# zsyOAOA/ResShift

Hardware: AMD Instinct MI355X
Metric: images/sec (1x3x64x64 LR -> 3x256x256, 15-step ResShift sampling loop incl. VQ encode/decode) (higher is better)
Workload: dtype f16x2 encoder + UNet (hi+lo fp16 pairs, 3 MFMAs per product: fp32-class) + f16 decoder (parity policy); 1 GPU; realsr_swinunet_realesrgan256: batch 32/GPU x 1 GPU, 1x3x64x64 LR -> 3x256x256, 15 steps, random-init weights; precision_policy=parity, parallelism=dp1 (batch sharded, one RCCL weight broadcast, no data-path collective)

## Files before the change

### include/resshift_hip.h

```cpp
#ifndef RESSHIFT_HIP_H
#define RESSHIFT_HIP_H
#include <stddef.h>
#include <stdint.h>

#ifdef __cplusplus
extern "C" {
#endif

#define RS_PREC_F16 0
#define RS_PREC_F32 1
#define RS_PREC_SPLIT 2
#define RS_MAX_LEVELS 8
#define RS_MAX_STEPS 64
#define RS_MAX_ROWS 64

typedef struct rs_engine rs_engine;

typedef struct rs_unet_config {
    int image_size, in_channels, model_channels, out_channels;
    int n_levels;
    int channel_mult[RS_MAX_LEVELS];
    int num_res_blocks[RS_MAX_LEVELS];
    int n_attn_res;
    int attention_resolutions[RS_MAX_LEVELS];
// ... 117 lines not shown
int rs_debug_enable(rs_engine* e, int on);
int rs_debug_count(rs_engine* e);
int rs_debug_info(rs_engine* e, int i, char* name, int name_cap, int* dims_bchw);
int rs_debug_fetch(rs_engine* e, int i, float* out_nchw_dev, void* stream);
int rs_debug_fetch_rows(rs_engine* e, int i, int b0, int nb, float* out_nchw_dev, void* stream);

int rs_op_conv2d(const void* x0, const void* x1, const float* w_ref_host, const float* bias_host, const void* res, void* y,
                 int B, int Hs, int Ws, int C0, int C1, int Cout, int KH, int KW, int stride, int pad_t, int pad_l, int Ho,
                 int Wo, int up, int act, int in_prec, int out_prec, int force_direct, void* stream);
int rs_op_conv2d_bench(const void* x0, const void* w_packed_dev, const float* bias_dev, const void* res, void* y, int B, int Hs,
                       int Ws, int Cin, int Cout, int KH, int KW, int stride, int pad, int Ho, int Wo, int up, int act, int in_prec,
                       int out_prec, int reps, float* ms_out, void* stream);
int rs_op_conv3x3_halo(const void* x, const float* coef_dev, int act_in, const float* w_ref_host, const float* bias_host, const void* res,
                       void* y, int B, int H, int W, int Cin, int Cout, int prec, float* ystats_dev, void* stream);
int rs_op_conv3x3_wino(const void* x, const float* coef_dev, int act_in, const float* w_ref_host, const float* bias_host, const void* res,
                       void* y, int B, int H, int W, int Cin, int Cout, float* ystats_dev, int reps, float* ms_out, void* stream);
int rs_op_conv3x3_halo_stats_px(int B, int H, int W, int Cin, int Cout, int prec);
int rs_op_gemm_nt(const void* a, const void* b, const float* bias_dev, void* y, int nz, int M, int N, int K, float scale,
                  int in_prec, int out_prec, void* stream);
int rs_op_groupnorm(const void* x, void* y, const float* gamma_host, const float* beta_host, const float* film_dev, int B, int HW,
                    int C, int groups, float eps, int act, int prec, void* stream);
int rs_op_window_attention(const void* qkv, void* out, const float* bias_table_host , int B, int H, int W,
                           int heads, int shift, int prec, void* stream);
int rs_op_window_attention_qkv(const void* x, const void* wqkv_dev, const float* bqkv_dev, const void* wproj_dev, const float* bproj_dev,
                               const void* res, void* out, const float* table_host, int B, int H, int W, int heads, int shift, void* stream);
int rs_op_window_attention_qkv_split(const void* x, const void* wqkv_dev, const float* bqkv_dev, const void* wproj_dev, const float* bproj_dev,
                                     const void* res, void* out, const float* table_host, const float* xcoef_dev, int B, int H, int W, int heads,
                                     int shift, void* stream);
int rs_op_ae_flash_attention(const void* q, const void* k, const void* vt, const float* bv_dev, void* o, int nz, int T, int C, void* stream);
int rs_op_ae_flash_attention_split(const void* q, const void* k, const void* vt, const float* bv_dev, void* o, int nz, int T, int C, void* stream);
int rs_op_swin_mlp(const void* x, const void* w1_dev, const float* b1_dev, const void* w2_dev, const float* b2_dev, const void* res, void* y,
// ... 16 lines not shown
```

### resshift_amd/_lib.py

```python
from __future__ import annotations

import ctypes as C
import os

import torch

HERE = os.path.dirname(os.path.abspath(__file__))
LIB_PATH = os.environ.get("RESSHIFT_HIP_LIB") or os.path.join(HERE, "libresshift_hip.so")

RS_PREC_F16 = 0
RS_PREC_F32 = 1
RS_PREC_SPLIT = 2
RS_MAX_LEVELS = 8
RS_MAX_STEPS = 64
RS_MAX_ROWS = 64


class UNetConfig(C.Structure):
    _fields_ = [
        ("image_size", C.c_int), ("in_channels", C.c_int), ("model_channels", C.c_int), ("out_channels", C.c_int),
        ("n_levels", C.c_int),
        ("channel_mult", C.c_int * RS_MAX_LEVELS),
        ("num_res_blocks", C.c_int * RS_MAX_LEVELS),
        ("n_attn_res", C.c_int),
# ... 100 lines not shown
    "rs_arena_bytes": (_SZ, [_P]),
    "rs_last_launch_count": (_LL, [_P]),
    "rs_profile_enable": (_I, [_P, _I]),
    "rs_profile_get": (_I, [_P, C.POINTER(C.c_double)]),
    "rs_profile_families": (_I, [_P, C.POINTER(C.c_double), _I]),
    "rs_profile_shapes": (_I, [_P, C.c_char_p, _I]),
    "rs_debug_enable": (_I, [_P, _I]),
    "rs_debug_count": (_I, [_P]),
    "rs_debug_info": (_I, [_P, _I, C.c_char_p, _I, C.POINTER(C.c_int)]),
    "rs_debug_fetch": (_I, [_P, _I, _P, _P]),
    "rs_debug_fetch_rows": (_I, [_P, _I, _I, _I, _P, _P]),
    "rs_op_conv2d": (_I, [_P, _P, _P, _P, _P, _P] + [_I] * 18 + [_P]),
    "rs_op_conv2d_bench": (_I, [_P, _P, _P, _P, _P] + [_I] * 16 + [C.POINTER(C.c_float), _P]),
    "rs_op_conv3x3_halo_stats_px": (_I, [_I, _I, _I, _I, _I, _I]),
    "rs_op_conv3x3_halo": (_I, [_P, _P, _I, _P, _P, _P, _P, _I, _I, _I, _I, _I, _I, _P, _P]),
    "rs_op_conv3x3_wino": (_I, [_P, _P, _I, _P, _P, _P, _P, _I, _I, _I, _I, _I, _P, _I, C.POINTER(C.c_float), _P]),
    "rs_op_gemm_nt": (_I, [_P, _P, _P, _P, _I, _I, _I, _I, _F, _I, _I, _P]),
    "rs_op_groupnorm": (_I, [_P, _P, _P, _P, _P, _I, _I, _I, _I, _F, _I, _I, _P]),
    "rs_op_window_attention": (_I, [_P, _P, _P, _I, _I, _I, _I, _I, _I, _P]),
    "rs_op_window_attention_qkv": (_I, [_P, _P, _P, _P, _P, _P, _P, _P, _I, _I, _I, _I, _I, _P]),
    "rs_op_window_attention_qkv_split": (_I, [_P, _P, _P, _P, _P, _P, _P, _P, _P, _I, _I, _I, _I, _I, _P]),
    "rs_op_swin_mlp": (_I, [_P, _P, _P, _P, _P, _P, _P, _I, _I, _I, _P]),
    "rs_op_ae_flash_attention": (_I, [_P, _P, _P, _P, _P, _I, _I, _I, _P]),
    "rs_op_ae_flash_attention_split": (_I, [_P, _P, _P, _P, _P, _I, _I, _I, _P]),
    "rs_op_swin_mlp_split": (_I, [_P, _P, _P, _P, _P, _P, _P, _I, _I, _I, _P]),
    "rs_op_swin_mlp_split_unembed": (_I, [_P, _P, _P, _P, _P, _P, _P, _I, _I, _I, _I, _I, _P]),
    "rs_op_softmax_rows": (_I, [_P, _P, _LL, _I, _I, _P]),
    "rs_op_vq": (_I, [_P, _P, _P, _P, _LL, _I, _I, _P]),
    "rs_op_nchw_to_nhwc": (_I, [_P, _P, _I, _I, _I, _I, _P]),
    "rs_op_nhwc_to_nchw": (_I, [_P, _P, _I, _I, _I, _I, _P]),
    "rs_op_convert": (_I, [_P, _I, _P, _I, _I, _LL, _P]),
# ... 100 lines not shown
```

### resshift_amd/csrc/engine.hip

```cpp
#include "common.h"
#include "../../include/resshift_hip.h"
#include <dlfcn.h>
#include <algorithm>
#include <array>
#include <cmath>
#include <cstdio>
#include <cstring>
#include <functional>
#include <map>
#include <string>
#include <unordered_map>
#include <vector>

extern "C" {
int rs_igemm_launch(const IGemmParams* p, int in_dt, int out_dt, int nz, hipStream_t st);
int rs_igemm_splitk_plan(int M, int Cout, int Ktot, int in_dt);
int rs_igemm4_pick(const IGemmParams* p, int in_dt, int out_dt, int nz, int* TW, int* BC);
int rs_igemm4_plan(const IGemmParams* p, int in_dt, int out_dt, int nz, int* TW, int* BC, int* SEG, int* SK);
int rs_igemm4_stats_px(const IGemmParams* p, int in_dt);
int rs_wino_plan(const IGemmParams* p, int in_dt, int out_dt, int nz);
int rs_wino_launch(const IGemmParams* p, hipStream_t st);
size_t rs_wino_weight_bytes(int Cin, int Cout);
float rs_wino_pack(const float* w_ref, int Cin, int Cout, void* dst);
int rs_wino_stats_px();
int rs_wino_tiles(const IGemmParams* p);
int rs_igemm_split_stats_px(const IGemmParams* p, int splitk);
int rs_direct_conv_launch(const DirectConvParams* p, int in_dt, int out_dt, hipStream_t st);
int rs_head_conv_launch(const void* x, int in_dt, const float* coef_dev, const float* w_dev, const float* bias_dev, float* y, int B, int H, int W, int C,
                        int ldx, int Cout, int ldy, hipStream_t st);
int rs_groupnorm_launch(const GNParams* p, int dt, int apply_slabs, hipStream_t st);
int rs_win_attn_launch(const WinAttnParams* p, int dt, hipStream_t st);
int rs_softmax_rows_launch(const float* s, void* out, int out_dt, long long nrows, int ncols, long long lds_, long long ldo, hipStream_t st);
int rs_nchw_to_nhwc_launch(const float* in, void* out, int out_dt, int B, int C, int HW, int ldo, int coff, float scale, hipStream_t st);
int rs_nhwc_to_nchw_launch(const void* in, int in_dt, float* out, int B, int C, int HW, int ldi, int coff, hipStream_t st);
int rs_axpbypcz_launch(const float* x, const float* z, const float* n, float* y, float a, float b, float c, long long cnt, hipStream_t st);
int rs_axpbypcz_rows_launch(const float* x, const float* z, const float* n, float* y, const float* a, const float* b, const float* c, long long per,
                            int B, hipStream_t st);
int rs_axpbypcz_seeded_launch(const float* x, const float* z, float* y, const float* a, const float* b, const float* c, const rs_noise_key* keys,
                              const rs_noise_key* keys_dev, const int* draw, long long per, int B, hipStream_t st);
// ... 410 lines not shown
                HostTensor t;
                if (d->second(t)) it = host.emplace(k, std::move(t)).first;
            }
        }
        if (it == host.end()) { if (build_err.empty()) build_err = "missing state_dict key: " + k; return nullptr; }
        return &it->second;
    }
    float* add_f32(const std::string& key, size_t n) {
        return (float*)blob.add(n * sizeof(float), [&](char* dst) {
            const HostTensor* t = find(key);
            if (!t) return;
            if (t->data.size() != n) { if (build_err.empty()) build_err = "bad size for " + key; return; }
            memcpy(dst, t->data.data(), n * sizeof(float));
        });
    }
    ConvW add_conv(const std::string& prefix, int Cin, int Cout, int KH, int KW, bool has_bias = true, bool force_direct = false, bool head = false) {
        ConvW c; c.Cin = Cin; c.Cout = Cout; c.KH = KH; c.KW = KW;
        c.idx = conv_count++;
        if ((int)big_w.size() < conv_count) big_w.resize(conv_count, 0);
        const int cidx = c.idx;
        c.direct = force_direct;
        c.CinP = c.direct ? Cin : (Cin + 7) / 8 * 8;
        const int CinP = c.CinP;
        const size_t K = (size_t)KH * KW * CinP, n = (size_t)KH * KW * Cin * Cout, np = K * Cout;
        const std::string wkey = prefix + ".weight";
        auto get = [&]() -> const float* {
            const HostTensor* t = find(wkey);
            if (!t) return nullptr;
            if (t->data.size() != n) { if (build_err.empty()) build_err = "bad size for " + wkey; return nullptr; }
            return t->data.data();
// ... 25 lines not shown
                    const float* w = get(); if (!w) return;
                    f16* o = (f16*)dst;
                    for (int co = 0; co < Cout; ++co)
                        for (int ci = 0; ci < Cin; ++ci)
                            for (int t = 0; t < KH * KW; ++t) {
                                f16 h, l;
                                const float wv = w[((size_t)co * Cin + ci) * KH * KW + t];
                                if (!std::isfinite(wv) || std::fabs(wv) > 60000.0f) { if (split_err.empty()) split_err = "split precision needs finite fp16-range weights: " + wkey; }
                                else if (!(std::fabs(wv) < 30.0f)) big_w[cidx] = 1;
                                rs_split(wv, h, l);
                                const size_t k = (size_t)t * CinP + ci;
                                o[(size_t)co * 2 * K + k] = h;
                                o[(size_t)co * 2 * K + K + k] = l;
                            }
                });
            static const bool wino_on = []() { const char* e = getenv("RS_WINO"); return !(e && e[0] == '0'); }();
            if (wino_on && cfg.enable_split && KH == 3 && KW == 3 && (Cin % 32) == 0 && Cin <= 640 && (Cout % 160) == 0 && Cout <= 320)
                c.ww = blob.add(rs_wino_weight_bytes(Cin, Cout), [&](char* dst) {
                    const float* w = get(); if (!w) return;
                    if (!(rs_wino_pack(w, Cin, Cout, dst) < 30.0f)) big_w[cidx] = 1;
                });
            if (cfg.enable_f32)
                c.wf = blob.add(np * 4, [&](char* dst) {
                    const float* w = get(); if (!w) return;
                    float* o = (float*)dst;
                    for (int co = 0; co < Cout; ++co)
                        for (int ci = 0; ci < Cin; ++ci)
                            for (int t = 0; t < KH * KW; ++t)
                                o[(size_t)co * K + (size_t)t * CinP + ci] = w[((size_t)co * Cin + ci) * KH * KW + t];
                });
        }
        if (head && !c.direct && KH == 3 && KW == 3 && Cout <= 4 && (Cin % 8) == 0)
// ... 242 lines not shown
        fe_out_ch = u.cond_lq ? base_chn : 0;
        int ch = u.channel_mult[0] * mc;
        const int input_ch = ch;
        {
            UBlock b; b.has_conv = true; b.level = 0; b.out_ch = ch;
            const bool two_src_unaligned = !fe_convs.empty() && (u.in_channels % 8 != 0);
            b.conv = add_conv("input_blocks.0.0", u.in_channels + fe_out_ch, ch, 3, 3, true, two_src_unaligned);
            in_blocks.push_back(b);
        }
        std::vector<int> chans{ch};
        int ds = u.image_size;
        for (int level = 0; level < u.n_levels; ++level) {
            const int mult = u.channel_mult[level];
            for (int jj = 0; jj < u.num_res_blocks[level]; ++jj) {
                UBlock b; b.level = level;
                const std::string p = "input_blocks." + std::to_string(in_blocks.size());
                b.has_res = true; b.res = add_resblock(p + ".0", ch, mult * mc, emb_ch);
                ch = mult * mc;
                if (in_attn_res(ds) && jj == 0) { b.has_swin = true; b.swin = add_basiclayer(p + ".1", ch, ds); }
                b.out_ch = ch;
                in_blocks.push_back(b); chans.push_back(ch);
            }
            if (level != u.n_levels - 1) {
                UBlock b; b.level = level + 1; b.has_down = true; b.out_ch = ch;
                b.conv = add_conv("input_blocks." + std::to_string(in_blocks.size()) + ".0.op", ch, ch, 3, 3);
                in_blocks.push_back(b); chans.push_back(ch);
                ds /= 2;
            }
        }
        skip_ch = chans;
        mid_res1 = add_resblock("middle_block.0", ch, ch, emb_ch);
        mid_swin = add_basiclayer("middle_block.1", ch, ds);
        mid_res2 = add_resblock("middle_block.2", ch, ch, emb_ch);
        for (int level = u.n_levels - 1; level >= 0; --level) {
            const int mult = u.channel_mult[level];
            for (int i = 0; i <= u.num_res_blocks[level]; ++i) {
                const int ich = chans.back(); chans.pop_back();
                UBlock b; b.level = level;
                const std::string p = "output_blocks." + std::to_string(out_blocks.size());
                h_ch.push_back(ch);
                int sub = 0;
                b.has_res = true; b.res = add_resblock(p + "." + std::to_string(sub++), ch + ich, mc * mult, emb_ch);
                ch = mc * mult;
                if (in_attn_res(ds) && i == 0) { b.has_swin = true; b.swin = add_basiclayer(p + "." + std::to_string(sub++), ch, ds); }
                if (level && i == u.num_res_blocks[level]) {
                    b.has_up = true;
                    b.conv = add_conv(p + "." + std::to_string(sub) + ".conv", ch, ch, 3, 3);
                    b.has_upf = add_upfold(p + "." + std::to_string(sub++) + ".conv", ch, b.upf);
                    ds *= 2;
                }
                b.out_ch = ch;
                out_blocks.push_back(b);
            }
        }
        out_norm = add_gn("out.0", ch);
        out_conv = add_conv("out.2", input_ch, u.out_channels, 3, 3, true, false, true);
    }
    ResBlockW add_resnet(const std::string& p, int Cin, int Cout) {
        ResBlockW r; r.Cin = Cin; r.Cout = Cout;
        r.n1 = add_gn(p + ".norm1", Cin);
        r.c1 = add_conv(p + ".conv1", Cin, Cout, 3, 3);
        r.n2 = add_gn(p + ".norm2", Cout);
        r.c2 = add_conv(p + ".conv2", Cout, Cout, 3, 3);
        r.has_skip = Cin != Cout;
        if (r.has_skip) r.skip = add_conv(p + ".nin_shortcut", Cin, Cout, 1, 1);
        return r;
    }
    AttnW add_attn(const std::string& p, int C) {
        AttnW a; a.C = C;
// ... 165 lines not shown
        if (!on || !fold || !r.has_skip || (X.dt != RS_F16S && !(X.dt == RS_F16 && on16)) || Y.dt != X.dt) return false;
        if (X.dt == RS_F16S && (big(r.skip) || big(r.c2))) return false;
        if (!r.skip.w_for(X.dt) || r.skip.KH != 1 || X.C != r.skip.CinP || (X.C % 32) || (X.ld % 8) || X.H != Y.H || X.W != Y.W) return false;
        int sk = 1, seg = 0;
        return halo_conv(r.c2, h1, Y, nullptr, &sk, &seg, true) && sk == 1 && seg == 0;
    }
    void want_stats(Exec& ex, const ConvW& w, const View& x, View& y, const View* res, int stride = 1, int pad = 1, int up = 1, bool folded = false) {
        static const bool on = []() { const char* e = getenv("RS_GN_EPI_STATS"); return !(e && e[0] == '0'); }();
        static const bool gen = []() { const char* e = getenv("RS_GN_GEN_STATS"); return !(e && e[0] == '0'); }();
        const int HW = y.H * y.W;
        y.st = nullptr; y.st2 = nullptr; y.st_prod = -1;
        if (!on || w.direct) return;
        const IGemmParams pp = conv_params(w, x, nullptr, y, stride, pad, pad, up, 0, res, 1.f);
        int spx = 0;
        bool wino = false;
        if (w.KH == 3 && stride == 1 && pad == 1 && up == 1 && halo_conv(w, x, y, res, nullptr, nullptr, folded, &wino)) spx = wino ? rs_wino_stats_px() : rs_igemm4_stats_px(&pp, x.dt);
        else if (gen && x.dt == RS_F16S && y.dt == RS_F16S && x.C == w.CinP)
            spx = rs_igemm_split_stats_px(&pp, rs_igemm_splitk_plan(pp.M, w.Cout, w.KH * w.KW * x.C, x.dt));
        if (spx <= 0 || (HW % spx)) return;
        y.stS = HW / spx; y.stld = y.C;
        y.st = ex.pool((size_t)y.B * y.stS * y.stld * 2 * sizeof(float));
        y.st_prod = ex.prod_seq++;
    }
    void gn_silu_conv3(Exec& ex, const GNW& g, const ConvW& w, const View& X, const View& Y, float eps, const float* film, const View* res,
                       const ConvW* skw = nullptr, const View* skx = nullptr) {
        static const bool fold = []() { const char* e = getenv("RS_GN_CONV_FOLD"); return !(e && e[0] == '0'); }();
        if (fold && halo_conv(w, X, Y, res, nullptr, nullptr, skw != nullptr)) {
            const float* coef = gn_coef(ex, g, X, eps, film);
            conv3(ex, w, X, Y, res, 0, coef, RS_ACT_SILU, skw, skx);
            return;
        }
// ... 1360 lines not shown
    if (!rs_igemm4_plan(&p, prec, prec, 1, &tw, &bc, &seg, &sk)) rc = fail("shape is not eligible for the halo kernel");
    else {
        p.splitk = sk;
        if (sk > 1) { (void)hipMalloc((void**)&part, (size_t)sk * p.M * Cout * sizeof(float)); p.partial = part; }
        p.ystats = ystats_dev; p.ystats_ld = Cout;
        rc = rs_igemm_launch(&p, prec, prec, 1, st);
    }
    (void)hipStreamSynchronize(st);
    if (part) (void)hipFree(part);
    if (wdev) (void)hipFree(wdev);
    if (bias) (void)hipFree(bias);
    return rc;
}

int rs_op_conv3x3_wino(const void* x, const float* coef_dev, int act_in, const float* w_ref_host, const float* bias_host, const void* res, void* y,
                       int B, int H, int W, int Cin, int Cout, float* ystats_dev, int reps, float* ms_out, void* stream) {
    hipStream_t st = (hipStream_t)stream;
    if (Cin < 32 || (Cin % 32) || Cout < 32 || (Cout % 32)) return fail("wino kernel: channels in multiples of 32");
    std::vector<char> packed(rs_wino_weight_bytes(Cin, Cout));
    const float mx = rs_wino_pack(w_ref_host, Cin, Cout, packed.data());
    if (!(mx < 30.0f)) return fail("wino kernel: |U| >= 30");
    void* wdev = dev_copy(packed.data(), packed.size());
    float* bias = bias_host ? (float*)dev_copy(bias_host, Cout * 4) : nullptr;
    IGemmParams p{};
    p.x0 = x; p.ww = wdev; p.bias = bias; p.res = res; p.y = y; p.C0 = Cin; p.ld0 = Cin; p.B = B; p.Hs = H; p.Ws = W; p.up = 1; p.Ho = H; p.Wo = W;
    p.KH = 3; p.KW = 3; p.stride = 1; p.pad_t = 1; p.pad_l = 1; p.Cout = Cout; p.ldy = Cout; p.ldres = Cout; p.M = B * H * W; p.Ktot = 9 * Cin;
    p.out_scale = 1.f; p.splitk = 1; p.xcoef = coef_dev; p.xact = act_in; p.ystats = ystats_dev; p.ystats_ld = Cout;
    int rc = 0;
    float* stamps = nullptr;
    const int ntile = rs_wino_tiles(&p);
    p.dbg = 64;
    if (const char* ab = getenv("RS_WINO_ABL")) p.dbg |= atoi(ab);
    if (getenv("RS_WINO_STAMPS")) { (void)hipMalloc((void**)&stamps, (size_t)ntile * 16 * sizeof(float)); (void)hipMemset(stamps, 0, (size_t)ntile * 16 * sizeof(float)); p.partial = stamps; }
    if (!rs_wino_plan(&p, RS_F16S, RS_F16S, 1)) rc = fail("shape is not eligible for the wino kernel");
    else {
        rc = rs_wino_launch(&p, st);
        if (rc) fail("wino launch failed");
        if (stamps) {
            (void)hipStreamSynchronize(st);
            std::vector<float> hs((size_t)ntile * 16);
            (void)hipMemcpy(hs.data(), stamps, hs.size() * sizeof(float), hipMemcpyDeviceToHost);
            double wide[16] = {}; int nw = 0;
            for (int t = 0; t < ntile; ++t) {
                for (int i = 0; i < 16; ++i) wide[i] += hs[(size_t)t * 16 + i];
                ++nw;
            }
// ... 203 lines not shown
```

### resshift_amd/csrc/wino.hip

```cpp
#include "igemm_common.h"
#include "gn_tail.h"
#include <algorithm>
#include <cmath>
#include <vector>

namespace {

using namespace igemm_detail;

typedef __attribute__((address_space(3))) void* lds_ptr_t;

__device__ __forceinline__ void wdma16s(__amdgpu_buffer_rsrc_t r, char* lds, unsigned voff, unsigned soff) {
    __builtin_amdgcn_raw_ptr_buffer_load_lds(r, (lds_ptr_t)lds, 16, voff, soff, 0, 0);
}

template <int N> __device__ __forceinline__ void wait_vm() { asm volatile("s_waitcnt vmcnt(%0)" ::"n"(N) : "memory"); }

constexpr int W_TH = 8, W_TW = 16;
constexpr int W_PITCH = 20;
constexpr int W_HROWS = (W_TH + 2) * W_PITCH;
constexpr int W_UPW = 2;
constexpr int W_NUNIT = 8 * W_UPW;
constexpr int W_HBUF = W_NUNIT * 2048;
constexpr int W_NBUF = 3;
constexpr int W_COEF = W_NBUF * W_HBUF;
constexpr int W_MAXCIN = 640;
constexpr int W_LDS = 160 * 1024;
static_assert(W_COEF + W_MAXCIN * 8 <= W_LDS && W_COEF + 8 * 1024 <= W_LDS, "LDS");
constexpr unsigned W_INV = 0xF0000000u;
__host__ __device__ constexpr int w_depth_of(int CF) { return CF <= 8 ? 4 : 2; }

__host__ __device__ constexpr int w_first(int i) { return i == 0 ? 0 : 1; }
__host__ __device__ constexpr int w_second(int i) { return i == 3 ? 3 : 2; }
__host__ __device__ constexpr float w_tau(int i) { return i == 1 ? 1.f : -1.f; }
__host__ __device__ constexpr float w_sigma(int i) { return i == 2 ? -1.f : 1.f; }
__host__ __device__ constexpr int w_cf_of(int Cout) { return (Cout % 160) == 0 ? 10 : ((Cout % 128) == 0 ? 8 : 4); }

#ifdef RS_WINO_PHASES
#define WSTAMP(i) do { const long long t_ = __builtin_readcyclecounter(); ph[i] += t_ - tprev; tprev = t_; } while (0)
#define WABL(bit) (p.dbg & (bit))
#else
#define WSTAMP(i) do {} while (0)
#define WABL(bit) false
#endif

template <int CF>
__global__ __launch_bounds__(512, 2) void wino_kernel(IGemmParams p) {
    constexpr int W_DEPTH = w_depth_of(CF);
    static_assert(CF % W_DEPTH == 0, "register slots for the weight fragments: the slot of a step is cf % W_DEPTH");
    constexpr int BC = 16 * CF, CFH = CF / 2;
    extern __shared__ __attribute__((aligned(16))) char smem[];
    const int tid = threadIdx.x, lane = tid & 63;
    const int wave = __builtin_amdgcn_readfirstlane(tid >> 6);
#ifdef RS_WINO_PHASES
    long long ph[16] = {0, 0, 0, 0, 0, 0, 0, 0, 0, 0, 0, 0, 0, 0, 0, 0};
    long long tprev = __builtin_readcyclecounter();
    const long long tstart = tprev;
#endif
    const int nby = p.Cout / BC;
    const int txb_n = p.Wo / W_TW, tyb_n = p.Ho / W_TH;
    int tile = xcd_remap(blockIdx.x, gridDim.x);
    const int nb = tile % nby; tile /= nby;
// ... 109 lines not shown
        const float tb = tau_b[pp];
#pragma unroll
        for (int half = 0; half < 2; ++half) {
            f32x4 px[4];
#pragma unroll
            for (int k = 0; k < 4; ++k) px[k] = *(const f32x4*)(q + (half ? (ax[pp][k] ^ 16) : ax[pp][k]));
#pragma unroll
            for (int e = 0; e < 4; ++e) {
                const float v = fmaf(fmaf(px[3][e], tb, px[2][e]), tau_a, fmaf(px[1][e], tb, px[0][e]));
                f16 hh, ll;
                rs_split(v, hh, ll); h[4 * half + e] = hh; l[4 * half + e] = ll;
            }
        }
    };

    f32x4 acc[2][2][CF];
#pragma unroll
    for (int pp = 0; pp < 2; ++pp)
#pragma unroll
        for (int tf = 0; tf < 2; ++tf)
#pragma unroll
            for (int i = 0; i < CF; ++i) acc[pp][tf][i] = f32x4{0.f, 0.f, 0.f, 0.f};

    if (xcoef) {
        const __amdgpu_buffer_rsrc_t rc = __builtin_amdgcn_make_buffer_rsrc((void*)(xcoef + (long long)b * 2 * Cin), 0, 2 * Cin * 4, 0x00020000);
        wdma16s(rc, smem + W_COEF + wave * 1024, (unsigned)(wave * 1024 + lane * 16), 0u);
    }
    issue_halo(0, 0);
    issue_halo(1, 1);
    f16x8 wh[W_DEPTH], wl[W_DEPTH];
    __builtin_amdgcn_sched_barrier(0);
#pragma unroll
    for (int s = 0; s < W_DEPTH; ++s) load_w(0, 0, 0, s, wh[s], wl[s]);
    __builtin_amdgcn_sched_barrier(0);
    wait_vm<2 * W_UPW + 2 * W_DEPTH>();
// ... 3 lines not shown
    convert_chunk(0, 0);
    WSTAMP(0);

    int buf = 0;
    for (int c = 0; c < nch; ++c) {
        wait_vm<2 * W_DEPTH>();
        asm volatile("s_waitcnt lgkmcnt(0)" ::: "memory");
        __builtin_amdgcn_s_barrier();
        asm volatile("" ::: "memory");
        WSTAMP(1);
        const int buf1 = buf == 2 ? 0 : buf + 1, buf2 = buf1 == 2 ? 0 : buf1 + 1;
        issue_halo(c + 2, buf2);
        WSTAMP(2);
#pragma unroll
        for (int pp = 0; pp < 2; ++pp) {
            f16x8 bh[2], bl[2];
            if (WABL(2)) { bh[0] = bh[1] = bl[0] = bl[1] = wh[0]; }
            else {
#pragma unroll
                for (int tf = 0; tf < 2; ++tf) { make_b(pp, tf, bh[tf], bl[tf]); __builtin_amdgcn_sched_barrier(0); }
            }
            WSTAMP(3);
#pragma unroll
            for (int cf = 0; cf < CF; ++cf) {
                const f16x8 ah = wh[cf % W_DEPTH], al = wl[cf % W_DEPTH];
                const f16x8 as = ah * (f16)RS_LO_SCALE;
                if (WABL(1)) { acc[pp][0][cf][0] += (float)(as[0] * bh[0][0] + al[1] * bl[1][1]); }
                else {
#pragma unroll
                    for (int tf = 0; tf < 2; ++tf) acc[pp][tf][cf] = __builtin_amdgcn_mfma_f32_16x16x32_f16(as, bh[tf], acc[pp][tf][cf], 0, 0, 0);
#pragma unroll
                    for (int tf = 0; tf < 2; ++tf) acc[pp][tf][cf] = __builtin_amdgcn_mfma_f32_16x16x32_f16(ah, bl[tf], acc[pp][tf][cf], 0, 0, 0);
#pragma unroll
                    for (int tf = 0; tf < 2; ++tf) acc[pp][tf][cf] = __builtin_amdgcn_mfma_f32_16x16x32_f16(al, bh[tf], acc[pp][tf][cf], 0, 0, 0);
                }
                __builtin_amdgcn_sched_barrier(0);
                if (!WABL(8)) load_w(c, pp, cf, W_DEPTH, wh[cf % W_DEPTH], wl[cf % W_DEPTH]);
                __builtin_amdgcn_sched_barrier(0);
            }
            WSTAMP(4);
        }
        if (c + 1 < nch && !WABL(4)) convert_chunk(c + 1, buf1);
        WSTAMP(5);
        {
            const int flip = buf == 2 ? -2 * W_HBUF : W_HBUF;
#pragma unroll
            for (int pp = 0; pp < 2; ++pp)
#pragma unroll
                for (int k = 0; k < 4; ++k) ax[pp][k] += flip;
// ... 20 lines not shown
    long long tq = __builtin_readcyclecounter();
#define WQ(i) do { const long long t_ = __builtin_readcyclecounter(); ph[i] += t_ - tq; tq = t_; } while (0)
#else
#define WQ(i) do {} while (0)
#endif
    if (!WABL(16)) {
#pragma unroll
    for (int half = 0; half < 2; ++half) {
        const int nc = n0 + half * CFH * 16 + oct * 8;
        f32x4 bv0 = {0.f, 0.f, 0.f, 0.f}, bv1 = bv0;
        if (p.bias && item) { bv0 = *(const f32x4*)(p.bias + nc); bv1 = *(const f32x4*)(p.bias + nc + 4); }
        float s1[8], s2[8];
#pragma unroll
        for (int e = 0; e < 8; ++e) s1[e] = s2[e] = 0.f;
#pragma unroll
        for (int tf = 0; tf < 2; ++tf) {
            asm volatile("s_waitcnt lgkmcnt(0)" ::: "memory");
            __builtin_amdgcn_s_barrier();
            asm volatile("" ::: "memory");
            WQ(9);
#pragma unroll
            for (int pp = 0; pp < 2; ++pp)
#pragma unroll
                for (int cq = 0; cq < CFH; ++cq)
                    *(f32x4*)(smem + ((4 * pi + 2 * jp + (pp ^ pflip)) * 16 + (lane & 15)) * TS + (cq * 16 + 4 * (lane >> 4)) * 4) = acc[pp][tf][half * CFH + cq];
            const int ty = 2 * tf + ((tl >> 3) & 1), tx = tl & 7;
            const long long m0 = ((long long)b * p.Ho + y0 + 2 * ty + yy) * p.Wo + x0 + 2 * tx;
            uint4 rh[2] = {uint4{0u, 0u, 0u, 0u}, uint4{0u, 0u, 0u, 0u}}, rl[2] = {uint4{0u, 0u, 0u, 0u}, uint4{0u, 0u, 0u, 0u}};
            if (res && item) {
#pragma unroll
                for (int x = 0; x < 2; ++x) {
// ... 83 lines not shown
        if (wave == 0) { const bool last = rs_gn_tail_arrive(p.tail, b); if (lane == 0) *tail_flag = last ? 1u : 0u; }
        __syncthreads();
        if (*tail_flag) rs_gn_tail_finish<512>(p.tail, b, (float*)smem);
    }
    }
#ifdef RS_WINO_PHASES
    WSTAMP(6);
    ph[7] = tprev - tstart;
    if (tid == 0 && p.partial) {
#pragma unroll
        for (int i = 0; i < 16; ++i) p.partial[(size_t)blockIdx.x * 16 + i] = (float)ph[i];
    }
#endif
}

template <int CF> hipError_t wino_launch_cf(const IGemmParams& p, int tiles, hipStream_t st) {
    static RsAttrFlags attr_flags;
    if (attr_flags.need()) (void)hipFuncSetAttribute((const void*)wino_kernel<CF>, hipFuncAttributeMaxDynamicSharedMemorySize, W_LDS);
    hipLaunchKernelGGL((wino_kernel<CF>), dim3(tiles), dim3(512), W_LDS, st, p);
    return hipGetLastError();
}

}

extern "C" size_t rs_wino_weight_bytes(int Cin, int Cout) { return (size_t)Cin * Cout * 64; }

extern "C" float rs_wino_pack(const float* w, int Cin, int Cout, void* dst_) {
    f16* dst = (f16*)dst_;
    static const double G[4][3] = {{1, 0, 0}, {.5, .5, .5}, {.5, -.5, .5}, {0, 0, 1}};
    const int nch = Cin / 32, CF = w_cf_of(Cout), BC = 16 * CF;
    float mx = 0.f;
    for (int n = 0; n < Cout; ++n) {
        const int nb = n / BC, nl = n - nb * BC, cf = nl / 16, lr = nl & 15;
        const size_t blk = (size_t)nb * 16 * nch * CF * 1024;
// ... 8 lines not shown
            for (int i = 0; i < 4; ++i)
                for (int j = 0; j < 4; ++j) {
                    const double u = (t[i][0] * G[j][0] + t[i][1] * G[j][1] + t[i][2] * G[j][2]) * (double)(w_sigma(i) * w_sigma(j));
                    const float uf = (float)u;
                    mx = std::max(mx, std::fabs(uf));
                    f16 h, l;
                    rs_split(uf, h, l);
                    const size_t o = blk + ((((size_t)(4 * i + j) * nch + c) * CF + cf) * 2) * 512 + (size_t)lane * 8 + e;
                    dst[o] = h; dst[o + 512] = l;
                }
        }
    }
    return mx;
}

extern "C" int rs_wino_plan(const IGemmParams* pp, int in_dt, int out_dt, int nz) {
    static const int on = []() { const char* e = getenv("RS_WINO"); return e ? atoi(e) : 1; }();
    static const int min_tiles = []() { const char* e = getenv("RS_WINO_MINTILES"); return e ? atoi(e) : 192; }();
    const IGemmParams& p = *pp;
    if (!on || in_dt != RS_F16S || out_dt != RS_F16S || nz != 1 || !p.ww || p.C1 != 0 || p.no_halo || p.sx || p.act != RS_ACT_NONE) return 0;
    if (p.KH != 3 || p.KW != 3 || p.stride != 1 || p.pad_t != 1 || p.pad_l != 1 || p.up != 1 || p.Ho != p.Hs || p.Wo != p.Ws || p.osc == 2) return 0;
    if ((p.C0 % 32) || p.C0 > W_MAXCIN || (p.ld0 % 8) || (p.Cout % (16 * w_cf_of(p.Cout))) || (p.ldy % 8) || (p.res && (p.ldres % 8))) return 0;
    if ((p.Ho % W_TH) || (p.Wo % W_TW) || p.splitk > 1) return 0;
    const long long tiles = (long long)p.B * (p.Ho / W_TH) * (p.Wo / W_TW) * (p.Cout / (16 * w_cf_of(p.Cout)));
    return (tiles >= min_tiles || (p.dbg & 64)) ? 1 : 0;
}

extern "C" int rs_wino_stats_px() { return W_TH * W_TW; }
extern "C" int rs_wino_tiles(const IGemmParams* p) { return p->B * (p->Ho / W_TH) * (p->Wo / W_TW) * (p->Cout / (16 * w_cf_of(p->Cout))); }

extern "C" int rs_wino_launch(const IGemmParams* pp, hipStream_t st) {
    if (!rs_wino_plan(pp, RS_F16S, RS_F16S, 1)) return -2;
    IGemmParams p = *pp;
    if (((size_t)p.x0 & 15) || ((size_t)p.y & 15) || ((size_t)p.res & 15) || ((size_t)p.ww & 15)) return -2;
    const size_t xb = (size_t)p.B * p.Hs * p.Ws * p.ld0 * 4;
    if (xb >= 0xF0000000ull) return -2;
    p.x_bytes = (unsigned)xb;
    const int CF = w_cf_of(p.Cout), nby = p.Cout / (16 * CF), per_image = (p.Ho / W_TH) * (p.Wo / W_TW);
    if (p.tail.coef) {
        if (!p.ystats) return -2;
        if (p.tail.C > 2048 || p.tail.groups < 1 || p.tail.groups > 64 || (p.tail.C % p.tail.groups)) return -2;
        p.tail.expected = per_image * nby;
        p.tail.st0 = p.ystats; p.tail.S0 = per_image; p.tail.ld0 = p.ystats_ld; p.tail.n0 = p.Cout;
    }
    const int tiles = p.B * per_image * nby;
    const hipError_t e = CF == 10 ? wino_launch_cf<10>(p, tiles, st) : (CF == 8 ? wino_launch_cf<8>(p, tiles, st) : wino_launch_cf<4>(p, tiles, st));
    return e == hipSuccess ? 0 : -1;
}
```

### resshift_amd/ops.py

```python
from __future__ import annotations

import ctypes as C

import torch

from . import _lib

F16, F32, SPLIT = _lib.RS_PREC_F16, _lib.RS_PREC_F32, _lib.RS_PREC_SPLIT


def _dt(prec: int) -> torch.dtype:
    return {F16: torch.float16, F32: torch.float32, SPLIT: torch.int32}[prec]


def _prec_of(t: torch.Tensor) -> int:
    return {torch.float16: F16, torch.float32: F32, torch.int32: SPLIT}[t.dtype]


def convert(x, prec):
    lib = _lib.load()
    x = x.contiguous()
    Cc = x.shape[-1]
    out = torch.empty(x.shape, device=x.device, dtype=_dt(prec))
    _lib.check(lib.rs_op_convert(x.data_ptr(), _prec_of(x), out.data_ptr(), prec, Cc, x.numel() // Cc, _lib.current_stream_ptr()), "convert")
# ... 39 lines not shown
    wh, wp = _hostf(w_ref)
    bh, bp = _hostf(bias) if bias is not None else (None, None)
    st = None
    if want_stats:
        spx = lib.rs_op_conv3x3_halo_stats_px(B, H, W, Cin, Cout, prec)
        if spx <= 0:
            raise RuntimeError("this shape gets no output statistics from the halo kernel")
        st = torch.zeros(B, (H * W) // spx, Cout, 2, device=x.device, dtype=torch.float32)
    rc = lib.rs_op_conv3x3_halo(x.data_ptr(), coef.data_ptr() if coef is not None else None, act_in, wp, bp,
                                res.data_ptr() if res is not None else None, y.data_ptr(), B, H, W, Cin, Cout, prec,
                                st.data_ptr() if st is not None else None, _lib.current_stream_ptr())
    _lib.check(rc, "rs_op_conv3x3_halo")
    return (y, st) if want_stats else y


def conv3x3_wino(x, w_ref, bias=None, coef=None, act_in=0, res=None, want_stats=False, reps=0):
    lib = _lib.load()
    B, H, W, Cin = x.shape
    Cout = w_ref.shape[0]
    if _prec_of(x) != 2:
        raise RuntimeError("the wino kernel takes split storage")
    y = torch.empty(B, H, W, Cout, device=x.device, dtype=x.dtype)
    wh, wp = _hostf(w_ref)
    bh, bp = _hostf(bias) if bias is not None else (None, None)
    st = torch.zeros(B, (H * W) // 128, Cout, 2, device=x.device, dtype=torch.float32) if want_stats else None
    ms = C.c_float(0.0)
    rc = lib.rs_op_conv3x3_wino(x.data_ptr(), coef.data_ptr() if coef is not None else None, act_in, wp, bp,
                                res.data_ptr() if res is not None else None, y.data_ptr(), B, H, W, Cin, Cout,
                                st.data_ptr() if st is not None else None, reps, C.byref(ms), _lib.current_stream_ptr())
    _lib.check(rc, "rs_op_conv3x3_wino")
    out = (y, st) if want_stats else y
    return (out, ms.value) if reps > 0 else out


def gemm_nt(a, b, bias=None, scale=1.0, out_prec=None):
    lib = _lib.load()
    in_prec = _prec_of(a)
    out_prec = in_prec if out_prec is None else out_prec
    nz, M, K = a.shape
    N = b.shape[1]
    y = torch.empty(nz, M, N, device=a.device, dtype=_dt(out_prec))
    rc = lib.rs_op_gemm_nt(a.data_ptr(), b.data_ptr(), bias.data_ptr() if bias is not None else None, y.data_ptr(), nz, M, N, K,
                           float(scale), in_prec, out_prec, _lib.current_stream_ptr())
    _lib.check(rc, "rs_op_gemm_nt")
# ... 182 lines not shown
```

### resshift_amd/sharding.py

```python
from __future__ import annotations

import math
import os
from typing import Callable, Sequence, Tuple

import torch
import torch.distributed as dist

from . import _lib


def free_port() -> int:
    import socket

    with socket.socket(socket.AF_INET, socket.SOCK_STREAM) as s:
        s.bind(("127.0.0.1", 0))
        return int(s.getsockname()[1])


def pick_backend(world: int) -> str:
    forced = os.environ.get("RESSHIFT_DIST_BACKEND")
    if forced:
        return forced
    if not torch.cuda.is_available():
# ... 109 lines not shown
    micro = math.ceil(n_global / world)
    pad = torch.zeros((micro,) + tuple(local.shape[1:]), dtype=local.dtype, device=local.device)
    pad[: local.shape[0]] = local
    parts = [torch.empty_like(pad) for _ in range(world)]
    dist.all_gather(parts, pad)
    return torch.cat(parts, 0)[:n_global]


def reflect_pad(x: torch.Tensor, pad_h: int, pad_w: int) -> torch.Tensor:
    H, W = x.shape[-2:]
    if pad_h >= H or pad_w >= W:
        raise ValueError("reflect padding must be smaller than the padded side (as torch.nn.functional.pad requires)")
    return _lib.window_copy(x, 0, 0, H + pad_h, W + pad_w)


BLOB_CACHE_MAGIC = b"RSBLOB06"
BLOB_CACHE_HEADER = 40


def checkpoint_fingerprint(paths) -> bytes:
    import hashlib

    h = hashlib.sha256()
    for p in paths or ():
        if p is None:
            h.update(b"<none>")
            continue
        p = os.path.abspath(str(p))
        h.update(p.encode())
        try:
            st = os.stat(p)
# ... 84 lines not shown
```

Baseline: 136.2 images/sec.

## Add half-height Winograd tiles and extend Winograd conv to wider, lower-resolution layers

The Winograd 3x3 conv kernel gets a template parameter for tile height, so a half-height variant (4 rows, 16 cols) can produce more tiles for small feature maps. Eligibility widens to Cout up to 640 on low-resolution UNet planes, and a new planner picks full or half tiles. The minimum-tile threshold is relaxed when the halo igemm path would not run unsplit. The intent is to move more 3x3 convs onto the Winograd path with enough parallelism, at the cost of less weight reuse per tile and a new blob cache version.

```diff
diff --git a/include/resshift_hip.h b/include/resshift_hip.h
--- a/include/resshift_hip.h
+++ b/include/resshift_hip.h
@@ -155,7 +155,7 @@
 int rs_op_conv3x3_halo(const void* x, const float* coef_dev, int act_in, const float* w_ref_host, const float* bias_host, const void* res,
                        void* y, int B, int H, int W, int Cin, int Cout, int prec, float* ystats_dev, void* stream);
 int rs_op_conv3x3_wino(const void* x, const float* coef_dev, int act_in, const float* w_ref_host, const float* bias_host, const void* res,
-                       void* y, int B, int H, int W, int Cin, int Cout, float* ystats_dev, int reps, float* ms_out, void* stream);
+                       void* y, int B, int H, int W, int Cin, int Cout, float* ystats_dev, int reps, float* ms_out, void* stream, int half_tiles);
 int rs_op_conv3x3_halo_stats_px(int B, int H, int W, int Cin, int Cout, int prec);
 int rs_op_gemm_nt(const void* a, const void* b, const float* bias_dev, void* y, int nz, int M, int N, int K, float scale,
                   int in_prec, int out_prec, void* stream);
diff --git a/resshift_amd/_lib.py b/resshift_amd/_lib.py
--- a/resshift_amd/_lib.py
+++ b/resshift_amd/_lib.py
@@ -138,7 +138,7 @@
     "rs_op_conv2d_bench": (_I, [_P, _P, _P, _P, _P] + [_I] * 16 + [C.POINTER(C.c_float), _P]),
     "rs_op_conv3x3_halo_stats_px": (_I, [_I, _I, _I, _I, _I, _I]),
     "rs_op_conv3x3_halo": (_I, [_P, _P, _I, _P, _P, _P, _P, _I, _I, _I, _I, _I, _I, _P, _P]),
-    "rs_op_conv3x3_wino": (_I, [_P, _P, _I, _P, _P, _P, _P, _I, _I, _I, _I, _I, _P, _I, C.POINTER(C.c_float), _P]),
+    "rs_op_conv3x3_wino": (_I, [_P, _P, _I, _P, _P, _P, _P, _I, _I, _I, _I, _I, _P, _I, C.POINTER(C.c_float), _P, _I]),
     "rs_op_gemm_nt": (_I, [_P, _P, _P, _P, _I, _I, _I, _I, _F, _I, _I, _P]),
     "rs_op_groupnorm": (_I, [_P, _P, _P, _P, _P, _I, _I, _I, _I, _F, _I, _I, _P]),
     "rs_op_window_attention": (_I, [_P, _P, _P, _I, _I, _I, _I, _I, _I, _P]),
diff --git a/resshift_amd/csrc/engine.hip b/resshift_amd/csrc/engine.hip
--- a/resshift_amd/csrc/engine.hip
+++ b/resshift_amd/csrc/engine.hip
@@ -19,10 +19,11 @@
 int rs_igemm4_plan(const IGemmParams* p, int in_dt, int out_dt, int nz, int* TW, int* BC, int* SEG, int* SK);
 int rs_igemm4_stats_px(const IGemmParams* p, int in_dt);
 int rs_wino_plan(const IGemmParams* p, int in_dt, int out_dt, int nz);
+int rs_wino_packs(int Cin, int Cout);
 int rs_wino_launch(const IGemmParams* p, hipStream_t st);
 size_t rs_wino_weight_bytes(int Cin, int Cout);
 float rs_wino_pack(const float* w_ref, int Cin, int Cout, void* dst);
-int rs_wino_stats_px();
+int rs_wino_stats_px(const IGemmParams* p);
 int rs_wino_tiles(const IGemmParams* p);
 int rs_igemm_split_stats_px(const IGemmParams* p, int splitk);
 int rs_direct_conv_launch(const DirectConvParams* p, int in_dt, int out_dt, hipStream_t st);
@@ -463,6 +464,7 @@
             memcpy(dst, t->data.data(), n * sizeof(float));
         });
     }
+    int wino_plane = 0;
     ConvW add_conv(const std::string& prefix, int Cin, int Cout, int KH, int KW, bool has_bias = true, bool force_direct = false, bool head = false) {
         ConvW c; c.Cin = Cin; c.Cout = Cout; c.KH = KH; c.KW = KW;
         c.idx = conv_count++;
@@ -518,8 +520,7 @@
                                 o[(size_t)co * 2 * K + K + k] = l;
                             }
                 });
-            static const bool wino_on = []() { const char* e = getenv("RS_WINO"); return !(e && e[0] == '0'); }();
-            if (wino_on && cfg.enable_split && KH == 3 && KW == 3 && (Cin % 32) == 0 && Cin <= 640 && (Cout % 160) == 0 && Cout <= 320)
+            if (cfg.enable_split && KH == 3 && KW == 3 && rs_wino_packs(Cin, Cout) && (Cout <= 320 || (wino_plane >= 16 && wino_plane % 16 == 0)))
                 c.ww = blob.add(rs_wino_weight_bytes(Cin, Cout), [&](char* dst) {
                     const float* w = get(); if (!w) return;
                     if (!(rs_wino_pack(w, Cin, Cout, dst) < 30.0f)) big_w[cidx] = 1;
@@ -792,6 +793,7 @@
             const int mult = u.channel_mult[level];
             for (int jj = 0; jj < u.num_res_blocks[level]; ++jj) {
                 UBlock b; b.level = level;
+                wino_plane = ds;
                 const std::string p = "input_blocks." + std::to_string(in_blocks.size());
                 b.has_res = true; b.res = add_resblock(p + ".0", ch, mult * mc, emb_ch);
                 ch = mult * mc;
@@ -807,6 +809,7 @@
             }
         }
         skip_ch = chans;
+        wino_plane = ds;
         mid_res1 = add_resblock("middle_block.0", ch, ch, emb_ch);
         mid_swin = add_basiclayer("middle_block.1", ch, ds);
         mid_res2 = add_resblock("middle_block.2", ch, ch, emb_ch);
@@ -815,6 +818,7 @@
             for (int i = 0; i <= u.num_res_blocks[level]; ++i) {
                 const int ich = chans.back(); chans.pop_back();
                 UBlock b; b.level = level;
+                wino_plane = ds;
                 const std::string p = "output_blocks." + std::to_string(out_blocks.size());
                 h_ch.push_back(ch);
                 int sub = 0;
@@ -831,6 +835,7 @@
                 out_blocks.push_back(b);
             }
         }
+        wino_plane = 0;
         out_norm = add_gn("out.0", ch);
         out_conv = add_conv("out.2", input_ch, u.out_channels, 3, 3, true, false, true);
     }
@@ -1026,7 +1031,7 @@
         const IGemmParams pp = conv_params(w, x, nullptr, y, stride, pad, pad, up, 0, res, 1.f);
         int spx = 0;
         bool wino = false;
-        if (w.KH == 3 && stride == 1 && pad == 1 && up == 1 && halo_conv(w, x, y, res, nullptr, nullptr, folded, &wino)) spx = wino ? rs_wino_stats_px() : rs_igemm4_stats_px(&pp, x.dt);
+        if (w.KH == 3 && stride == 1 && pad == 1 && up == 1 && halo_conv(w, x, y, res, nullptr, nullptr, folded, &wino)) spx = wino ? rs_wino_stats_px(&pp) : rs_igemm4_stats_px(&pp, x.dt);
         else if (gen && x.dt == RS_F16S && y.dt == RS_F16S && x.C == w.CinP)
             spx = rs_igemm_split_stats_px(&pp, rs_igemm_splitk_plan(pp.M, w.Cout, w.KH * w.KW * x.C, x.dt));
         if (spx <= 0 || (HW % spx)) return;
@@ -2417,7 +2422,7 @@
 }
 
 int rs_op_conv3x3_wino(const void* x, const float* coef_dev, int act_in, const float* w_ref_host, const float* bias_host, const void* res, void* y,
-                       int B, int H, int W, int Cin, int Cout, float* ystats_dev, int reps, float* ms_out, void* stream) {
+                       int B, int H, int W, int Cin, int Cout, float* ystats_dev, int reps, float* ms_out, void* stream, int half_tiles) {
     hipStream_t st = (hipStream_t)stream;
     if (Cin < 32 || (Cin % 32) || Cout < 32 || (Cout % 32)) return fail("wino kernel: channels in multiples of 32");
     std::vector<char> packed(rs_wino_weight_bytes(Cin, Cout));
@@ -2431,8 +2436,8 @@
     p.out_scale = 1.f; p.splitk = 1; p.xcoef = coef_dev; p.xact = act_in; p.ystats = ystats_dev; p.ystats_ld = Cout;
     int rc = 0;
     float* stamps = nullptr;
+    p.dbg = 64 | (half_tiles ? 128 : 0);
     const int ntile = rs_wino_tiles(&p);
-    p.dbg = 64;
     if (const char* ab = getenv("RS_WINO_ABL")) p.dbg |= atoi(ab);
     if (getenv("RS_WINO_STAMPS")) { (void)hipMalloc((void**)&stamps, (size_t)ntile * 16 * sizeof(float)); (void)hipMemset(stamps, 0, (size_t)ntile * 16 * sizeof(float)); p.partial = stamps; }
     if (!rs_wino_plan(&p, RS_F16S, RS_F16S, 1)) rc = fail("shape is not eligible for the wino kernel");
diff --git a/resshift_amd/csrc/wino.hip b/resshift_amd/csrc/wino.hip
--- a/resshift_amd/csrc/wino.hip
+++ b/resshift_amd/csrc/wino.hip
@@ -16,17 +16,15 @@
 
 template <int N> __device__ __forceinline__ void wait_vm() { asm volatile("s_waitcnt vmcnt(%0)" ::"n"(N) : "memory"); }
 
-constexpr int W_TH = 8, W_TW = 16;
+constexpr int W_TW = 16;
 constexpr int W_PITCH = 20;
-constexpr int W_HROWS = (W_TH + 2) * W_PITCH;
-constexpr int W_UPW = 2;
-constexpr int W_NUNIT = 8 * W_UPW;
+constexpr int W_NUNIT = 16;
 constexpr int W_HBUF = W_NUNIT * 2048;
 constexpr int W_NBUF = 3;
 constexpr int W_COEF = W_NBUF * W_HBUF;
 constexpr int W_MAXCIN = 640;
 constexpr int W_LDS = 160 * 1024;
-static_assert(W_COEF + W_MAXCIN * 8 <= W_LDS && W_COEF + 8 * 1024 <= W_LDS, "LDS");
+static_assert(W_COEF + W_MAXCIN * 8 <= W_LDS && W_COEF + 8 * 1024 <= W_LDS && W_MAXCIN * 8 <= 8 * 1024, "LDS");
 constexpr unsigned W_INV = 0xF0000000u;
 __host__ __device__ constexpr int w_depth_of(int CF) { return CF <= 8 ? 4 : 2; }
 
@@ -44,8 +42,9 @@
 #define WABL(bit) false
 #endif
 
-template <int CF>
+template <int CF, int TF>
 __global__ __launch_bounds__(512, 2) void wino_kernel(IGemmParams p) {
+    constexpr int W_TH = 4 * TF, W_UPW = TF, W_HROWS = (W_TH + 2) * W_PITCH;
     constexpr int W_DEPTH = w_depth_of(CF);
     static_assert(CF % W_DEPTH == 0, "register slots for the weight fragments: the slot of a step is cf % W_DEPTH");
     constexpr int BC = 16 * CF, CFH = CF / 2;
@@ -185,11 +184,11 @@
         }
     };
 
-    f32x4 acc[2][2][CF];
+    f32x4 acc[2][TF][CF];
 #pragma unroll
     for (int pp = 0; pp < 2; ++pp)
 #pragma unroll
-        for (int tf = 0; tf < 2; ++tf)
+        for (int tf = 0; tf < TF; ++tf)
 #pragma unroll
             for (int i = 0; i < CF; ++i) acc[pp][tf][i] = f32x4{0.f, 0.f, 0.f, 0.f};
 
@@ -223,25 +222,25 @@
         WSTAMP(2);
 #pragma unroll
         for (int pp = 0; pp < 2; ++pp) {
-            f16x8 bh[2], bl[2];
-            if (WABL(2)) { bh[0] = bh[1] = bl[0] = bl[1] = wh[0]; }
+            f16x8 bh[TF], bl[TF];
+            if (WABL(2)) { for (int tf = 0; tf < TF; ++tf) bh[tf] = bl[tf] = wh[0]; }
             else {
 #pragma unroll
-                for (int tf = 0; tf < 2; ++tf) { make_b(pp, tf, bh[tf], bl[tf]); __builtin_amdgcn_sched_barrier(0); }
+                for (int tf = 0; tf < TF; ++tf) { make_b(pp, tf, bh[tf], bl[tf]); __builtin_amdgcn_sched_barrier(0); }
             }
             WSTAMP(3);
 #pragma unroll
             for (int cf = 0; cf < CF; ++cf) {
                 const f16x8 ah = wh[cf % W_DEPTH], al = wl[cf % W_DEPTH];
                 const f16x8 as = ah * (f16)RS_LO_SCALE;
-                if (WABL(1)) { acc[pp][0][cf][0] += (float)(as[0] * bh[0][0] + al[1] * bl[1][1]); }
+                if (WABL(1)) { acc[pp][0][cf][0] += (float)(as[0] * bh[0][0] + al[1] * bl[TF - 1][1]); }
                 else {
 #pragma unroll
-                    for (int tf = 0; tf < 2; ++tf) acc[pp][tf][cf] = __builtin_amdgcn_mfma_f32_16x16x32_f16(as, bh[tf], acc[pp][tf][cf], 0, 0, 0);
-#pragma unroll
-                    for (int tf = 0; tf < 2; ++tf) acc[pp][tf][cf] = __builtin_amdgcn_mfma_f32_16x16x32_f16(ah, bl[tf], acc[pp][tf][cf], 0, 0, 0);
-#pragma unroll
-                    for (int tf = 0; tf < 2; ++tf) acc[pp][tf][cf] = __builtin_amdgcn_mfma_f32_16x16x32_f16(al, bh[tf], acc[pp][tf][cf], 0, 0, 0);
+                    for (int tf = 0; tf < TF; ++tf) acc[pp][tf][cf] = __builtin_amdgcn_mfma_f32_16x16x32_f16(as, bh[tf], acc[pp][tf][cf], 0, 0, 0);
+#pragma unroll
+                    for (int tf = 0; tf < TF; ++tf) acc[pp][tf][cf] = __builtin_amdgcn_mfma_f32_16x16x32_f16(ah, bl[tf], acc[pp][tf][cf], 0, 0, 0);
+#pragma unroll
+                    for (int tf = 0; tf < TF; ++tf) acc[pp][tf][cf] = __builtin_amdgcn_mfma_f32_16x16x32_f16(al, bh[tf], acc[pp][tf][cf], 0, 0, 0);
                 }
                 __builtin_amdgcn_sched_barrier(0);
                 if (!WABL(8)) load_w(c, pp, cf, W_DEPTH, wh[cf % W_DEPTH], wl[cf % W_DEPTH]);
@@ -292,7 +291,7 @@
 #pragma unroll
         for (int e = 0; e < 8; ++e) s1[e] = s2[e] = 0.f;
 #pragma unroll
-        for (int tf = 0; tf < 2; ++tf) {
+        for (int tf = 0; tf < TF; ++tf) {
             asm volatile("s_waitcnt lgkmcnt(0)" ::: "memory");
             __builtin_amdgcn_s_barrier();
             asm volatile("" ::: "memory");
@@ -406,10 +405,10 @@
 #endif
 }
 
-template <int CF> hipError_t wino_launch_cf(const IGemmParams& p, int tiles, hipStream_t st) {
+template <int CF, int TF> hipError_t wino_launch_cf(const IGemmParams& p, int tiles, hipStream_t st) {
     static RsAttrFlags attr_flags;
-    if (attr_flags.need()) (void)hipFuncSetAttribute((const void*)wino_kernel<CF>, hipFuncAttributeMaxDynamicSharedMemorySize, W_LDS);
-    hipLaunchKernelGGL((wino_kernel<CF>), dim3(tiles), dim3(512), W_LDS, st, p);
+    if (attr_flags.need()) (void)hipFuncSetAttribute((const void*)wino_kernel<CF, TF>, hipFuncAttributeMaxDynamicSharedMemorySize, W_LDS);
+    hipLaunchKernelGGL((wino_kernel<CF, TF>), dim3(tiles), dim3(512), W_LDS, st, p);
     return hipGetLastError();
 }
 
@@ -448,36 +447,57 @@
     return mx;
 }
 
+extern "C" int rs_wino_enabled() {
+    static const int on = []() { const char* e = getenv("RS_WINO"); return (e && e[0] == '0') ? 0 : 1; }();
+    return on;
+}
+extern "C" int rs_wino_packs(int Cin, int Cout) { return rs_wino_enabled() && (Cin % 32) == 0 && Cin <= W_MAXCIN && (Cout % 160) == 0 && Cout <= 640; }
+
+extern "C" int rs_igemm4_plan(const IGemmParams* pp, int in_dt, int out_dt, int nz, int* TW, int* BC, int* SEG, int* SK);
+
+constexpr int W_MINTILES = 192, W_MINTILES_SMALL = 128;
+static int wino_tf(const IGemmParams& p) {
+    if (p.Wo % W_TW) return 0;
+    const int nby = p.Cout / (16 * w_cf_of(p.Cout));
+    const bool full_ok = (p.Ho % 8) == 0, half_ok = (p.Ho % 4) == 0 && w_cf_of(p.Cout) == 10;
+    if (p.dbg & 64) return (p.dbg & 128) ? (half_ok ? 1 : 0) : (full_ok ? 2 : 0);
+    if (full_ok && (!half_ok || (long long)p.B * (p.Ho / 8) * (p.Wo / W_TW) * nby >= W_MINTILES)) return 2;
+    return half_ok ? 1 : 0;
+}
 extern "C" int rs_wino_plan(const IGemmParams* pp, int in_dt, int out_dt, int nz) {
-    static const int on = []() { const char* e = getenv("RS_WINO"); return e ? atoi(e) : 1; }();
-    static const int min_tiles = []() { const char* e = getenv("RS_WINO_MINTILES"); return e ? atoi(e) : 192; }();
+    static const int min_tiles = []() { const char* e = getenv("RS_WINO_MINTILES"); return e ? atoi(e) : -1; }();
     const IGemmParams& p = *pp;
-    if (!on || in_dt != RS_F16S || out_dt != RS_F16S || nz != 1 || !p.ww || p.C1 != 0 || p.no_halo || p.sx || p.act != RS_ACT_NONE) return 0;
+    if (!rs_wino_enabled() || in_dt != RS_F16S || out_dt != RS_F16S || nz != 1 || !p.ww || p.C1 != 0 || p.no_halo || p.sx || p.act != RS_ACT_NONE) return 0;
     if (p.KH != 3 || p.KW != 3 || p.stride != 1 || p.pad_t != 1 || p.pad_l != 1 || p.up != 1 || p.Ho != p.Hs || p.Wo != p.Ws || p.osc == 2) return 0;
     if ((p.C0 % 32) || p.C0 > W_MAXCIN || (p.ld0 % 8) || (p.Cout % (16 * w_cf_of(p.Cout))) || (p.ldy % 8) || (p.res && (p.ldres % 8))) return 0;
-    if ((p.Ho % W_TH) || (p.Wo % W_TW) || p.splitk > 1) return 0;
-    const long long tiles = (long long)p.B * (p.Ho / W_TH) * (p.Wo / W_TW) * (p.Cout / (16 * w_cf_of(p.Cout)));
-    return (tiles >= min_tiles || (p.dbg & 64)) ? 1 : 0;
-}
-
-extern "C" int rs_wino_stats_px() { return W_TH * W_TW; }
-extern "C" int rs_wino_tiles(const IGemmParams* p) { return p->B * (p->Ho / W_TH) * (p->Wo / W_TW) * (p->Cout / (16 * w_cf_of(p->Cout))); }
+    const int tf = wino_tf(p);
+    if (!tf || p.splitk > 1) return 0;
+    if (((size_t)p.x0 & 15) || ((size_t)p.y & 15) || ((size_t)p.res & 15) || ((size_t)p.ww & 15)) return 0;
+    if ((unsigned long long)p.B * p.Hs * p.Ws * p.ld0 * 4ull >= 0xF0000000ull) return 0;
+    if (p.tail.coef && (!p.ystats || p.tail.C > 2048 || p.tail.groups < 1 || p.tail.groups > 64 || (p.tail.C % p.tail.groups))) return 0;
+    if (p.dbg & 64) return 1;
+    const long long tiles = (long long)p.B * p.Ho * p.Wo / (8 * W_TW) * (p.Cout / (16 * w_cf_of(p.Cout)));
+    if (min_tiles >= 0) return tiles >= min_tiles ? 1 : 0;
+    int tw, bc, seg = 0, sk = 1;
+    const bool halo_full = rs_igemm4_plan(pp, in_dt, out_dt, nz, &tw, &bc, &seg, &sk) != 0 && sk == 1;
+    return tiles >= (halo_full ? W_MINTILES : W_MINTILES_SMALL) ? 1 : 0;
+}
+
+extern "C" int rs_wino_stats_px(const IGemmParams* p) { return 4 * wino_tf(*p) * W_TW; }
+extern "C" int rs_wino_tiles(const IGemmParams* p) { const int tf = wino_tf(*p); return tf ? p->B * (p->Ho / (4 * tf)) * (p->Wo / W_TW) * (p->Cout / (16 * w_cf_of(p->Cout))) : 0; }
 
 extern "C" int rs_wino_launch(const IGemmParams* pp, hipStream_t st) {
     if (!rs_wino_plan(pp, RS_F16S, RS_F16S, 1)) return -2;
     IGemmParams p = *pp;
-    if (((size_t)p.x0 & 15) || ((size_t)p.y & 15) || ((size_t)p.res & 15) || ((size_t)p.ww & 15)) return -2;
-    const size_t xb = (size_t)p.B * p.Hs * p.Ws * p.ld0 * 4;
-    if (xb >= 0xF0000000ull) return -2;
-    p.x_bytes = (unsigned)xb;
-    const int CF = w_cf_of(p.Cout), nby = p.Cout / (16 * CF), per_image = (p.Ho / W_TH) * (p.Wo / W_TW);
+    p.x_bytes = (unsigned)((size_t)p.B * p.Hs * p.Ws * p.ld0 * 4);
+    const int tf = wino_tf(p);
+    const int CF = w_cf_of(p.Cout), nby = p.Cout / (16 * CF), per_image = (p.Ho / (4 * tf)) * (p.Wo / W_TW);
     if (p.tail.coef) {
-        if (!p.ystats) return -2;
-        if (p.tail.C > 2048 || p.tail.groups < 1 || p.tail.groups > 64 || (p.tail.C % p.tail.groups)) return -2;
         p.tail.expected = per_image * nby;
         p.tail.st0 = p.ystats; p.tail.S0 = per_image; p.tail.ld0 = p.ystats_ld; p.tail.n0 = p.Cout;
     }
     const int tiles = p.B * per_image * nby;
-    const hipError_t e = CF == 10 ? wino_launch_cf<10>(p, tiles, st) : (CF == 8 ? wino_launch_cf<8>(p, tiles, st) : wino_launch_cf<4>(p, tiles, st));
+    const hipError_t e = tf == 1 ? wino_launch_cf<10, 1>(p, tiles, st)
+                                 : (CF == 10 ? wino_launch_cf<10, 2>(p, tiles, st) : (CF == 8 ? wino_launch_cf<8, 2>(p, tiles, st) : wino_launch_cf<4, 2>(p, tiles, st)));
     return e == hipSuccess ? 0 : -1;
 }
diff --git a/resshift_amd/ops.py b/resshift_amd/ops.py
--- a/resshift_amd/ops.py
+++ b/resshift_amd/ops.py
@@ -77,7 +77,7 @@
     return (y, st) if want_stats else y
 
 
-def conv3x3_wino(x, w_ref, bias=None, coef=None, act_in=0, res=None, want_stats=False, reps=0):
+def conv3x3_wino(x, w_ref, bias=None, coef=None, act_in=0, res=None, want_stats=False, reps=0, half_tiles=False):
     lib = _lib.load()
     B, H, W, Cin = x.shape
     Cout = w_ref.shape[0]
@@ -86,11 +86,11 @@
     y = torch.empty(B, H, W, Cout, device=x.device, dtype=x.dtype)
     wh, wp = _hostf(w_ref)
     bh, bp = _hostf(bias) if bias is not None else (None, None)
-    st = torch.zeros(B, (H * W) // 128, Cout, 2, device=x.device, dtype=torch.float32) if want_stats else None
+    st = torch.zeros(B, (H * W) // (64 if half_tiles else 128), Cout, 2, device=x.device, dtype=torch.float32) if want_stats else None
     ms = C.c_float(0.0)
     rc = lib.rs_op_conv3x3_wino(x.data_ptr(), coef.data_ptr() if coef is not None else None, act_in, wp, bp,
                                 res.data_ptr() if res is not None else None, y.data_ptr(), B, H, W, Cin, Cout,
-                                st.data_ptr() if st is not None else None, reps, C.byref(ms), _lib.current_stream_ptr())
+                                st.data_ptr() if st is not None else None, reps, C.byref(ms), _lib.current_stream_ptr(), 1 if half_tiles else 0)
     _lib.check(rc, "rs_op_conv3x3_wino")
     out = (y, st) if want_stats else y
     return (out, ms.value) if reps > 0 else out
diff --git a/resshift_amd/sharding.py b/resshift_amd/sharding.py
--- a/resshift_amd/sharding.py
+++ b/resshift_amd/sharding.py
@@ -147,7 +147,7 @@
     return _lib.window_copy(x, 0, 0, H + pad_h, W + pad_w)
 
 
-BLOB_CACHE_MAGIC = b"RSBLOB06"
+BLOB_CACHE_MAGIC = b"RSBLOB07"
 BLOB_CACHE_HEADER = 40
 
 
```

Measured after the change: 136.9 images/sec, median of 6. About the same (+0.5%).
